# ningyu1991/InclusiveGAN

Measured on AMD Instinct MI355X. Metric: training img/sec (whole node), CelebA 128x128 StyleGAN2+IMLE, higher is better.
Workload: dtype f32-equivalent (3x3 convs: 2-piece fp16 split, operands to <= 1 ulp of fp32, scales per pixel / per channel: no per-tensor window; fp32 sums)

## Files before the change

### inclusivegan_amd/csrc/conv2d_mfma.hip

```cpp
#include "igan_common.h"
#include <cmath>
#include <cstdlib>
#include <type_traits>

namespace {

typedef float f32x16 __attribute__((ext_vector_type(16)));

constexpr int BK = 32;
#ifndef IGAN_SPLIT
#define IGAN_SPLIT 8
#endif
constexpr int LDK = BK + 4;

struct ConvArgs {
    const float* x;
    const float* w;
    float* y;
    float* out;
    const float* in_scale;
    const float* out_scale;
    int N, H, W, Cin;
    int OH, OW, Cout;
    int KH, KW;
// ... 1234 lines not shown
    } else {
#pragma unroll
        for (int i = 0; i < 16; i++) v[i] = w[((size_t)tap * K + 16 * c + i) * Nn + n];
    }
    unsigned short pc[2][16];
#pragma unroll
    for (int i = 0; i < 16; i++) {
        unsigned short o[2];
        split2(v[i] * S, o);
        pc[0][i] = o[0]; pc[1][i] = o[1];
    }
    uint4* dst = reinterpret_cast<uint4*>(out + (((size_t)c * taps + tap) * Nn + n) * 32);
#pragma unroll
    for (int q = 0; q < 2; q++)
#pragma unroll
        for (int hh = 0; hh < 2; hh++) {
            uint4 u;
            u.x = pc[q][8 * hh + 0] | ((unsigned)pc[q][8 * hh + 1] << 16); u.y = pc[q][8 * hh + 2] | ((unsigned)pc[q][8 * hh + 3] << 16);
            u.z = pc[q][8 * hh + 4] | ((unsigned)pc[q][8 * hh + 5] << 16); u.w = pc[q][8 * hh + 6] | ((unsigned)pc[q][8 * hh + 7] << 16);
            dst[2 * q + hh] = u;
        }
}

template <int NP, bool TAPO = false>
__global__ __launch_bounds__(512, 4) void conv_fwd_planes_kernel(ConvArgs a) {
    constexpr int BM = 128, BN = 128, WN = 4, TM = 2;
    static_assert(NP == 3 || NP == 2, "three bf16 pieces (six products) or two fp16 pieces (three products)");
    constexpr int IMG = NP * 128 * 32, STAGE = 2 * IMG;
    constexpr unsigned PB = NP * 32u;
    constexpr int TABS = (NP == 2) ? 9 * BM * 4 : 0;
#ifndef IGAN_F16_LDS_PAD
#define IGAN_F16_LDS_PAD 0
#endif
    constexpr int LPAD = (NP == 2) ? IGAN_F16_LDS_PAD : 0;
    __shared__ __attribute__((aligned(1024))) unsigned char smem[P_NSTAGE * STAGE + 3 * BM * 4 + TABS + LPAD];
    int* row_pix = reinterpret_cast<int*>(smem + P_NSTAGE * STAGE);
    int* row_n = row_pix + BM;
    float* row_nz = reinterpret_cast<float*>(row_n + BM);
    float* tab_s = row_nz + BM;

#ifdef IGAN_DIAGNOSTIC
    const int dm = a.diag_mode;
    if (dm & 4) return;
#else
    constexpr int dm = 0;
#endif
// ... 641 lines not shown
    const float alpha = (a.splits == 1) ? a.alpha : 1.0f;
#pragma unroll
    for (int tm = 0; tm < TM; tm++) {
#pragma unroll
        for (int r = 0; r < 16; r++) {
            const int cir = m0 + wm * (BM / WM) + tile_row<TM, true>(tm, (r & 3) + 8 * (r >> 2) + 4 * h);
            if (cir >= a.Cin) continue;
            if constexpr (TN == 2) {
                if (a.vecY) {
                    const int c2 = cbase + 2 * l31;
                    if (c2 < a.Cout) *reinterpret_cast<float2*>(out + (size_t)cir * a.Cout + c2) = make_float2(acc[tm][0][r] * alpha, acc[tm][1][r] * alpha);
                    continue;
                }
            }
#pragma unroll
            for (int tn = 0; tn < TN; tn++) {
                const int cc = cbase + tile_row<TN, true>(tn, l31);
                if (cc < a.Cout) out[(size_t)cir * a.Cout + cc] = acc[tm][tn][r] * alpha;
            }
        }
    }
}

__global__ __launch_bounds__(256, 2) void conv_fwd_planes_w4_kernel(ConvArgs a) {
    constexpr int BM = 128, BN = 128, NS = 3;
    constexpr int IMG = 2 * 128 * 32, STAGE = 2 * IMG;
    constexpr unsigned PB = 64u;
    constexpr int TABS = 9 * BM * 4;
    __shared__ __attribute__((aligned(1024))) unsigned char smem[NS * STAGE + 3 * BM * 4 + TABS];
    int* row_pix = reinterpret_cast<int*>(smem + NS * STAGE);
    int* row_n = row_pix + BM;
    float* row_nz = reinterpret_cast<float*>(row_n + BM);
    float* tab_s = row_nz + BM;

    const int tid = threadIdx.x;
    const int lane = tid & 63, wave = __builtin_amdgcn_readfirstlane(tid >> 6);
    const int l31 = lane & 31, h = lane >> 5;
    const int wm = wave >> 1, wn = wave & 1;
    const int up = 1 << a.up_shift;
    auto stamp = [&](int k) {
        if (a.diag != nullptr && (threadIdx.x >> 6) == 0) {
            const unsigned long long t = __builtin_amdgcn_s_memrealtime();
            if ((threadIdx.x & 63) == 0) a.diag[(size_t)blockIdx.x * 4 + k] = t;
        }
    };
    stamp(0);
    int bid = blockIdx.x;
    if (a.xcd_remap && bid < a.full_tiles) {
        const int per_class = a.nx * a.ny;
        const int lo = (bid / per_class) * per_class;
        const int cnt = min(per_class, a.full_tiles - lo);
        bid = lo + remap_xcd(bid - lo, cnt);
        if (cnt == per_class && a.ny > 1 && a.stride > 1) {
            const int j = bid - lo;
            bid = lo + (j % a.ny) * a.nx + j / a.ny;
        }
    }
    const bool sliced = bid >= a.full_tiles;
    const int tail = bid - a.full_tiles;
    const int tile = sliced ? a.full_tiles + tail / a.splits : bid;
    const int split = sliced ? tail % a.splits : 0;
    const int nsplit = sliced ? a.splits : 1;
    const int mt = tile % a.nx, nt = (tile / a.nx) % a.ny, cls = tile / (a.nx * a.ny);
    const int py = cls >> a.up_shift, px = cls & (up - 1);
    const int QH = (a.OH - py + up - 1) >> a.up_shift;
    const int QW = (a.OW - px + up - 1) >> a.up_shift;
    const int Mcls = a.N * QH * QW;
    const int m0 = mt * BM;
    if (m0 >= Mcls) return;
    const int n0 = nt * BN;
    const int ky0 = (a.pad_y - py * a.stride) & (up - 1);
    const int kx0 = (a.pad_x - px * a.stride) & (up - 1);
    const int nky = (ky0 < a.KH) ? ((a.KH - ky0 + up - 1) >> a.up_shift) : 0;
    const int nkx = (kx0 < a.KW) ? ((a.KW - kx0 + up - 1) >> a.up_shift) : 0;
    const int chunks = nky * nkx * a.cpt;
    const int c_begin = sliced ? (int)(((long long)split * chunks) / nsplit) : 0;
    const int c_end = sliced ? (int)(((long long)(split + 1) * chunks) / nsplit) : chunks;
    const bool any = c_begin < c_end;

    const float inv_hw = 1.0f / (float)(QH * QW), inv_w = 1.0f / (float)QW;
    const int drow = 32 * wave + (lane >> 1);
    const int dhalf = (lane & 1) ^ ((drow >> 3) & 1);
    const int ntap = nky * nkx;
    int ld_t0 = any ? c_begin / a.cpt : 0;
    int ld_cc = any ? c_begin - ld_t0 * a.cpt : 0;
    int ld_ta = any ? ld_t0 / nkx : 0;
    int ld_tb = any ? ld_t0 - ld_ta * nkx : 0;
    const unsigned xbytes = (unsigned)a.N * a.H * a.W * a.Cin * 4u, wbytes = (unsigned)a.KH * a.KW * a.Cin * a.Cout * 4u;
    const __amdgpu_buffer_rsrc_t rx = __builtin_amdgcn_make_buffer_rsrc(const_cast<unsigned short*>(a.xp), 0, (int)xbytes, 0x00020000);
    const __amdgpu_buffer_rsrc_t rw = __builtin_amdgcn_make_buffer_rsrc(const_cast<unsigned short*>(a.wp), 0, (int)wbytes, 0x00020000);
    const unsigned pixA = (unsigned)a.Cin * 4u;
    unsigned baseA, maskA = 0u, voffB;
    {
        const int m = m0 + drow;
        const bool rok = m < Mcls;
        const int mm = rok ? m : 0;
        const int nn = div_small(mm, QH * QW, inv_hw);
        const int r = mm - nn * (QH * QW);
        const int qy = div_small(r, QW, inv_w), qx = r - qy * QW;
        const int vy0 = (qy * up + py) * a.stride - a.pad_y + ky0, vx0 = (qx * up + px) * a.stride - a.pad_x + kx0;
        const int iy0 = vy0 >> a.up_shift, ix0 = vx0 >> a.up_shift;
        baseA = (unsigned)((nn * a.H + iy0) * a.W + ix0) * pixA + (unsigned)dhalf * 16u;
        for (int ta = 0; ta < nky; ta++)
            for (int tb = 0; tb < nkx; tb++) {
                const int iy = iy0 + ta, ix = ix0 + tb;
                const bool ok = rok & (iy >= 0) & (ix >= 0) & (iy < a.H) & (ix < a.W);
                maskA |= ok ? (1u << (ta * nkx + tb)) : 0u;
            }
        const int co = n0 + drow;
        voffB = (co < a.Cout) ? (unsigned)co * PB + (unsigned)dhalf * 16u : OOB;
    }
    unsigned offA = OOB, soffB = 0u;
    typedef __attribute__((address_space(3))) void lds_void;
    bool dma_fresh = true;
    const unsigned sliceB = (unsigned)(a.KH * a.KW * a.Cout) * PB;
    auto dma_prep = [&]() {
        if (dma_fresh || ld_cc == 0) {
            const unsigned disp = (unsigned)(ld_ta * a.W + ld_tb) * pixA + (unsigned)ld_cc * PB;
            const unsigned bit = 1u << (ld_ta * nkx + ld_tb);
            offA = (maskA & bit) ? baseA + disp : OOB;
            const int ky = ky0 + (ld_ta << a.up_shift), kx = kx0 + (ld_tb << a.up_shift);
            soffB = __builtin_amdgcn_readfirstlane((unsigned)((ld_cc * (a.KH * a.KW) + ky * a.KW + kx) * a.Cout) * PB);
            dma_fresh = false;
        } else {
            offA += PB;
            soffB = __builtin_amdgcn_readfirstlane(soffB + sliceB);
        }
        ++ld_cc;
        const int w1 = (ld_cc == a.cpt) ? 1 : 0;
        ld_cc = w1 ? 0 : ld_cc;
        ld_tb += w1;
        const int w2 = (ld_tb == nkx) ? 1 : 0;
        ld_tb = w2 ? 0 : ld_tb;
// ... 9 lines not shown
            __builtin_amdgcn_raw_ptr_buffer_load_lds(rw, (lds_void*)(D + IMG), 16, voffB, sB, 0, 0);
            __builtin_amdgcn_raw_ptr_buffer_load_lds(rw, (lds_void*)(D + IMG + 4096), 16, voffB, sB + 32u, 0, 0);
        }
    };

    f32x16 acc[2][2];
#pragma unroll
    for (int i = 0; i < 2; i++)
#pragma unroll
        for (int j = 0; j < 2; j++)
#pragma unroll
            for (int r = 0; r < 16; r++) acc[i][j][r] = 0.0f;

    float tabv[5] = {0.0f, 0.0f, 0.0f, 0.0f, 0.0f};
    {
        const float* rowinv = reinterpret_cast<const float*>(reinterpret_cast<const unsigned char*>(a.xp) + (size_t)a.N * a.H * a.W * a.Cin * 4);
#pragma unroll
        for (int j = 0; j < 5; j++) {
            const int i = tid + 256 * j;
            const int t = i >> 7, r = i & 127;
            if (t < ntap) {
                const int ta = t / nkx, tb = t - ta * nkx;
                const int m = m0 + r;
                const bool rok = m < Mcls;
                const int mm = rok ? m : 0;
                const int nn = div_small(mm, QH * QW, inv_hw);
                const int rr = mm - nn * (QH * QW);
                const int qy = div_small(rr, QW, inv_w), qx = rr - qy * QW;
                const int iy = (((qy * up + py) * a.stride - a.pad_y + ky0) >> a.up_shift) + ta, ix = (((qx * up + px) * a.stride - a.pad_x + kx0) >> a.up_shift) + tb;
                if (rok & (iy >= 0) & (ix >= 0) & (iy < a.H) & (ix < a.W)) tabv[j] = rowinv[(nn * a.H + iy) * a.W + ix];
            }
        }
    }
    if (any) {
#pragma unroll
        for (int j = 0; j < 3; j++) { dma_prep(); dma_pair(j, 0); dma_pair(j, 1); }
    }
#pragma unroll
    for (int j = 0; j < 5; j++)
        if (tid + 256 * j < 9 * BM) tab_s[tid + 256 * j] = tabv[j];
    if (tid < BM) {
        const int m = m0 + tid;
        int pix = -1, nn = 0;
        if (m < Mcls) {
            nn = div_small(m, QH * QW, inv_hw);
            const int r = m - nn * (QH * QW);
            const int qy = div_small(r, QW, inv_w), qx = r - qy * QW;
            pix = (nn * a.OH + (qy * up + py)) * a.OW + (qx * up + px);
        }
        row_pix[tid] = pix;
        row_n[tid] = nn;
        row_nz[tid] = noise_term(a, pix);
    }
    const unsigned lds0 = (unsigned)(unsigned long long)(lds_void*)smem;
    const int ra = wm * 64 + l31, rb = wn * 64 + l31;
    const unsigned fa = lds0 + (unsigned)(2 * ra + (h ^ ((ra >> 3) & 1))) * 16u;
    const unsigned fb = lds0 + (unsigned)IMG + (unsigned)(2 * rb + (h ^ ((rb >> 3) & 1))) * 16u;
    stamp(1);

    const f32x16 zero = {0.f, 0.f, 0.f, 0.f, 0.f, 0.f, 0.f, 0.f, 0.f, 0.f, 0.f, 0.f, 0.f, 0.f, 0.f, 0.f};
    struct Frag { f16x8 a0[2], a1[2], b0[2], b1[2]; };
    auto read_frags = [&](Frag& f, int stage) {
        const unsigned va = fa + (unsigned)(stage * STAGE), vb = fb + (unsigned)(stage * STAGE);
        asm volatile("ds_read_b128 %0, %1" : "=v"(f.b0[0]) : "v"(vb));
        asm volatile("ds_read_b128 %0, %1" : "=v"(f.a0[0]) : "v"(va));
        asm volatile("ds_read_b128 %0, %1 offset:4096" : "=v"(f.b1[0]) : "v"(vb));
        asm volatile("ds_read_b128 %0, %1 offset:5120" : "=v"(f.b1[1]) : "v"(vb));
// ... 75 lines not shown
#pragma unroll
                for (int r = 0; r < 16; r++) { u[0][j][r] = 0.0f; u[1][j][r] = 0.0f; }
            }
            cs = 0; ++ct;
            const int tn_ = min(ct, ntap - 1);
            sc0 = tab_row[tn_ * BM]; sc1 = tab_row[tn_ * BM + 32];
        }
        st = st1;
    };
    if (any) {
        asm volatile("s_waitcnt vmcnt(8) lgkmcnt(0)\n\ts_barrier" ::: "memory");
        read_frags(F0, 0);
        sc0 = tab_row[ct * BM]; sc1 = tab_row[ct * BM + 32];
        int c = c_begin;
        for (; c + 1 < c_end; c += 2) { step(F0, F1, c, std::false_type()); step(F1, F0, c + 1, std::false_type()); }
        if (c < c_end) step(F0, F1, c, std::true_type());
        else
            asm volatile("s_waitcnt lgkmcnt(0)"
                         : "+v"(F0.a0[0]), "+v"(F0.a0[1]), "+v"(F0.a1[0]), "+v"(F0.a1[1]), "+v"(F0.b0[0]), "+v"(F0.b0[1]), "+v"(F0.b1[0]), "+v"(F0.b1[1]) :: "memory");
    }
    drain_lds_dma();
    stamp(2);
    const float* winv = reinterpret_cast<const float*>(reinterpret_cast<const unsigned char*>(a.wp) + (size_t)a.KH * a.KW * a.Cin * a.Cout * 4);
    if (sliced && nsplit > 1) {
        float* wst = a.y + ((size_t)(tile - a.full_tiles) * a.splits + split) * (BM * BN);
#pragma unroll
        for (int tn = 0; tn < 2; tn++) {
            const int cq = n0 + wn * 64 + tn * 32 + 4 * h;
            float4 wi[4];
#pragma unroll
            for (int q = 0; q < 4; q++) wi[q] = (cq + 8 * q < a.Cout) ? *reinterpret_cast<const float4*>(winv + cq + 8 * q) : f4zero();
#pragma unroll
            for (int tm = 0; tm < 2; tm++) {
                const int row = wm * 64 + tm * 32 + l31;
#pragma unroll
                for (int q = 0; q < 4; q++)
                    *reinterpret_cast<float4*>(wst + row * BN + wn * 64 + tn * 32 + 8 * q + 4 * h) =
                        make_float4(acc[tm][tn][4 * q] * wi[q].x, acc[tm][tn][4 * q + 1] * wi[q].y, acc[tm][tn][4 * q + 2] * wi[q].z, acc[tm][tn][4 * q + 3] * wi[q].w);
            }
        }
        return;
    }
    __syncthreads();
    const bool scale = a.out_scale != nullptr;
    const float alpha = a.alpha;
#pragma unroll
    for (int tn = 0; tn < 2; tn++) {
        const int cq = n0 + wn * 64 + tn * 32 + 4 * h;
        float4 wi[4], bia[4];
#pragma unroll
        for (int q = 0; q < 4; q++) {
            wi[q] = (cq + 8 * q < a.Cout) ? *reinterpret_cast<const float4*>(winv + cq + 8 * q) : f4zero();
            bia[q] = (a.act && a.bias && cq + 8 * q < a.Cout) ? *reinterpret_cast<const float4*>(a.bias + cq + 8 * q) : f4zero();
        }
#pragma unroll
        for (int tm = 0; tm < 2; tm++) {
            const int row = wm * 64 + tm * 32 + l31;
            const int pix = row_pix[row];
            if (pix < 0) continue;
            const float* osc = a.out_scale + (size_t)row_n[row] * a.Cout;
            const float nz = row_nz[row];
#pragma unroll
            for (int q = 0; q < 4; q++) {
                const int co = cq + 8 * q;
                if (co >= a.Cout) continue;
                float4 o = make_float4(acc[tm][tn][4 * q] * wi[q].x, acc[tm][tn][4 * q + 1] * wi[q].y, acc[tm][tn][4 * q + 2] * wi[q].z, acc[tm][tn][4 * q + 3] * wi[q].w);
                o.x *= alpha; o.y *= alpha; o.z *= alpha; o.w *= alpha;
                if (scale) { const float4 d = *reinterpret_cast<const float4*>(osc + co); o.x *= d.x; o.y *= d.y; o.z *= d.z; o.w *= d.w; }
                if (a.act) {
                    o.x = epi_act(a.act, o.x + nz + bia[q].x, a.act_alpha) * a.act_gain; o.y = epi_act(a.act, o.y + nz + bia[q].y, a.act_alpha) * a.act_gain;
                    o.z = epi_act(a.act, o.z + nz + bia[q].z, a.act_alpha) * a.act_gain; o.w = epi_act(a.act, o.w + nz + bia[q].w, a.act_alpha) * a.act_gain;
                }
                *reinterpret_cast<float4*>(a.out + (size_t)pix * a.Cout + co) = o;
            }
        }
    }
    stamp(3);
}

typedef __attribute__((ext_vector_type(4))) short s16x4;
#ifndef IGAN_WGRAD_ASM_DMA
#define IGAN_WGRAD_ASM_DMA 1
#endif
typedef unsigned u32x4 __attribute__((ext_vector_type(4)));
__device__ __forceinline__ u32x4 raw_rsrc_words(const void* base, unsigned bytes) {
    const unsigned long long b = (unsigned long long)(uintptr_t)base;
    u32x4 r;
    r[0] = __builtin_amdgcn_readfirstlane((unsigned)b);
    r[1] = __builtin_amdgcn_readfirstlane((unsigned)(b >> 32) & 0xFFFFu);
    r[2] = __builtin_amdgcn_readfirstlane(bytes);
    r[3] = 0x00020000u;
    return r;
}
template <int SOFF>
__device__ __forceinline__ void lds_dma16_asm(u32x4 rsrc, unsigned lds_addr, unsigned voffset) {
    asm volatile("s_mov_b32 m0, %0\n\ts_nop 0\n\tbuffer_load_dwordx4 %1, %2, %3 offen lds" ::"s"(lds_addr), "v"(voffset), "s"(rsrc), "n"(SOFF) : "memory", "m0");
}
template <int NP>
__global__ __launch_bounds__(512, 4) void conv_wgrad_planes_kernel(WgradArgs a) {
    constexpr int TM = 2, WN = 4;
    static_assert(NP == 3 || NP == 2, "three bf16 pieces (six products) or two fp16 pieces (three products)");
// ... 413 lines not shown
    hipLaunchKernelGGL(rows_f16_kernel, dim3(grid), dim3(256), 0, stream, x, scale, out, rowinv, colmax, total, cpp, ilog2(cpp), C, HW);
}
void launch_colmax_only(hipStream_t stream, const float* x, const float* scale, float* colmax, int P_, int HW, int C) {
    const int C4 = C / 4, ppi = 256 / C4;
    const int blocks = std::min(H_COLBLOCKS, igan::ceil_div(P_, ppi));
    hipLaunchKernelGGL(cols_amax_kernel, dim3(blocks), dim3(256), 0, stream, x, scale, colmax + 4, P_, C4, ilog2(C4), HW, colmax);
}
void launch_col_image(hipStream_t stream, const float* x, const float* scale, unsigned short* out, int P_, int HW, int C, const float* colmax) {
    const int cpp = C / PK, total = P_ * cpp, C4 = C / 4;
    float* inv = reinterpret_cast<float*>(reinterpret_cast<unsigned char*>(out) + (size_t)P_ * C * 4);
    float* sc = inv + C;
    float* partial = sc + C;
    const int ppi = 256 / C4;
    const int blocks = std::min(H_COLBLOCKS, igan::ceil_div(P_, ppi));
    if (colmax == nullptr) {
        hipLaunchKernelGGL(cols_amax_kernel, dim3(blocks), dim3(256), 0, stream, x, scale, partial, P_, C4, ilog2(C4), HW, (float*)nullptr);
        hipLaunchKernelGGL(cols_finalize_kernel, dim3(igan::ceil_div(C, 8)), dim3(256), 0, stream, (const float*)partial, inv, sc, blocks, C, (const float*)nullptr);
    } else
        hipLaunchKernelGGL(cols_finalize_kernel, dim3(igan::ceil_div(C, 8)), dim3(256), 0, stream, colmax + 4, inv, sc, 0, C, colmax);
    hipLaunchKernelGGL(cols_f16_kernel, dim3(igan::ceil_div(total, 256)), dim3(256), 0, stream, x, scale, out, (const float*)sc, total, cpp, C, HW);
}
bool f16_tap_outer() { static const int v = getenv("IGAN_F16_TAP_OUTER") ? atoi(getenv("IGAN_F16_TAP_OUTER")) : 1; return v != 0; }
bool f16_w4() { static const int v = getenv("IGAN_F16_W4") ? atoi(getenv("IGAN_F16_W4")) : 1; return v != 0; }
void launch_filter_image(hipStream_t stream, const float* w, unsigned short* wp, bool wt, int taps, int KW_, int Nn, int K) {
    const int wtotal = taps * Nn * (K / PK);
    if (planes_mode() == 2) {
        float* inv = reinterpret_cast<float*>(reinterpret_cast<unsigned char*>(wp) + (size_t)taps * Nn * K * 4);
        float* partial = inv + Nn;
        if (wt) {
            hipLaunchKernelGGL((filter_amax_kernel<true>), dim3(igan::ceil_div(taps * Nn, 4)), dim3(256), 0, stream, w, partial, taps, Nn, K);
            hipLaunchKernelGGL((filter_planes_f16_kernel<true>), dim3(igan::ceil_div(wtotal, 256)), dim3(256), 0, stream, w, wp, inv, (const float*)partial, taps, taps, KW_, Nn, K);
        } else {
            hipLaunchKernelGGL((filter_amax_kernel<false>), dim3(taps * H_KSK, igan::ceil_div(Nn, 64)), dim3(256), 0, stream, w, partial, taps, Nn, K);
            hipLaunchKernelGGL((filter_planes_f16_kernel<false>), dim3(igan::ceil_div(wtotal, 256)), dim3(256), 0, stream, w, wp, inv, (const float*)partial, taps * H_KSK, taps, KW_, Nn, K);
        }
    } else {
        if (wt) hipLaunchKernelGGL((filter_planes_kernel<true>), dim3(igan::ceil_div(wtotal, 256)), dim3(256), 0, stream, w, wp, taps, KW_, Nn, K);
        else hipLaunchKernelGGL((filter_planes_kernel<false>), dim3(igan::ceil_div(wtotal, 256)), dim3(256), 0, stream, w, wp, taps, KW_, Nn, K);
    }
}

bool planes_shape_ok(const igan_conv2d_params* p, const FwdTile& t, int Mmax) {
    if (!planes_enabled() || t.BM != 128 || t.BN != 128 || p->Cin % BK != 0) return false;
    static const int min_rows = getenv("IGAN_PLANES_MIN_ROWS") ? atoi(getenv("IGAN_PLANES_MIN_ROWS")) : 1024;
    if (p->KH * p->KW == 1 || (long long)p->KH * p->KW * p->Cin < 1152 || Mmax < min_rows) return false;
    if ((long long)p->N * p->OH * p->OW >= (1LL << 24)) return false;
    if ((long long)p->N * p->H * p->W * p->Cin * 6 >= 0x7FFFFF00LL || (long long)p->KH * p->KW * p->Cin * p->Cout * 6 >= 0x7FFFFF00LL) return false;
    if (planes_mode() == 2 && (!pow2(p->Cin / PK) || p->Cin / PK > 64 || p->KH * p->KW > 9 || p->Cout % 4 != 0)) return false;
#ifdef IGAN_DIAGNOSTIC
    {
        static const int only_cin = getenv("IGAN_PLANES_ONLY_CIN") ? atoi(getenv("IGAN_PLANES_ONLY_CIN")) : 0;
        static const int no_act = getenv("IGAN_PLANES_NO_ACT") ? atoi(getenv("IGAN_PLANES_NO_ACT")) : 0;
        static const int no_scale = getenv("IGAN_PLANES_NO_SCALE") ? atoi(getenv("IGAN_PLANES_NO_SCALE")) : 0;
        static const int kind = getenv("IGAN_PLANES_KIND") ? atoi(getenv("IGAN_PLANES_KIND")) : 0;
        static const int wt = getenv("IGAN_PLANES_WT") ? atoi(getenv("IGAN_PLANES_WT")) : 0;
        if (only_cin && p->Cin != only_cin) return false;
        if ((no_act == 1 && p->act != 0) || (no_act == 2 && p->act == 0)) return false;
        if ((no_scale == 1 && p->in_scale != nullptr) || (no_scale == 2 && p->in_scale == nullptr)) return false;
        if ((kind == 1 && (p->stride != 1 || p->up != 1)) || (kind == 2 && p->stride != 2) || (kind == 3 && p->up != 2)) return false;
        if ((wt == 1 && p->w_transposed) || (wt == 2 && !p->w_transposed)) return false;
    }
#endif
    return true;
}
bool use_planes_kernel(const igan_conv2d_params* p, const FwdTile& t, int Mmax) {
    if (!planes_shape_ok(p, t, Mmax) || (((uintptr_t)p->x | (uintptr_t)p->w | (uintptr_t)p->in_scale | (uintptr_t)p->x_pieces) & 15) != 0) return false;
    if (planes_mode() == 2 && (((uintptr_t)p->y | (uintptr_t)p->out_scale | (uintptr_t)p->bias) & 15) != 0) return false;
    return true;
// ... 194 lines not shown
    if (planes) {
        IGAN_REQUIRE(p->x_pieces == nullptr || planes_mode() == 1, "conv2d: the two-piece fp16 form writes its own images (one scale per pixel here, per channel in the weight gradient): x_pieces must be NULL");
        IGAN_REQUIRE(p->x_pieces == nullptr || p->x_pieces_bytes == planes_x_floats(p) * 4, "conv2d: x_pieces is not the image of this x (x_pieces_bytes != N*H*W*Cin*6)");
        const unsigned short* xp = reinterpret_cast<const unsigned short*>(p->x_pieces);
        unsigned short* wp = reinterpret_cast<unsigned short*>(p->workspace + partial_floats + planes_x_floats(p));
        const int cpp = p->Cin / PK;
        if (xp == nullptr) {
            unsigned short* own = reinterpret_cast<unsigned short*>(p->workspace + partial_floats);
            if (a.diag_mode & 1) {}
            else if (planes_mode() == 2) launch_row_image(stream, p->x, p->in_scale, own, p->N * p->H * p->W, p->H * p->W, p->Cin, p->x_colmax);
            else launch_piece_image(stream, p->x, p->in_scale, own, p->N * p->H * p->W, p->H * p->W, p->Cin);
            xp = own;
        }
        if (p->w_pieces != nullptr) {
            IGAN_REQUIRE(p->w_pieces_bytes == igan_filter_image_bytes(p->KH, p->KW, p->Cin, p->Cout) && (((uintptr_t)p->w_pieces) & 15) == 0,
                         "conv2d: w_pieces is not an image igan_filter_image() wrote for this filter (size / alignment)");
            wp = reinterpret_cast<unsigned short*>(const_cast<void*>(p->w_pieces));
        } else if (!(a.diag_mode & 1)) launch_filter_image(stream, p->w, wp, wt, p->KH * p->KW, p->KW, p->Cout, p->Cin);
        a.xp = xp; a.wp = wp;
        a.cpt = cpp;
        if (a.diag_mode & 2) {}
        else if (planes_mode() == 2) {
            const bool tapo = f16_tap_outer();
            if (tapo && f16_w4()) hipLaunchKernelGGL(conv_fwd_planes_w4_kernel, grid, dim3(256), 0, stream, a);
            else if (tapo) hipLaunchKernelGGL((conv_fwd_planes_kernel<2, true>), grid, dim3(512), 0, stream, a);
            else hipLaunchKernelGGL((conv_fwd_planes_kernel<2, false>), grid, dim3(512), 0, stream, a);
        } else hipLaunchKernelGGL((conv_fwd_planes_kernel<3>), grid, dim3(512), 0, stream, a);
        IGAN_LAUNCH_CHECK("conv2d (piece form) launch");
        launched = true;
    } else
    if (use_dma_kernel(p, t, a.walk != 0)) {
        if (wt) {
            if (a.in_scale) hipLaunchKernelGGL((conv_fwd_dma_kernel<true, true>), grid, dim3(512), 0, stream, a);
            else hipLaunchKernelGGL((conv_fwd_dma_kernel<true, false>), grid, dim3(512), 0, stream, a);
        } else {
            if (a.in_scale) hipLaunchKernelGGL((conv_fwd_dma_kernel<false, true>), grid, dim3(512), 0, stream, a);
            else hipLaunchKernelGGL((conv_fwd_dma_kernel<false, false>), grid, dim3(512), 0, stream, a);
        }
        IGAN_LAUNCH_CHECK("conv2d (LDS-DMA) launch");
        launched = true;
    }
    if (launched) {}
    else if (t.BM == 128 && t.BN == 128 && eight_waves("IGAN_CONV_8WAVE")) launch_fwd<128, 128, 2, 4>(stream, a, grid, wt, vec);
    else if (t.BM == 128 && t.BN == 128) launch_fwd<128, 128, 2, 2>(stream, a, grid, wt, vec);
    else if (t.BM == 128 && t.BN == 64 && eight_waves("IGAN_CONV_8WAVE")) launch_fwd<128, 64, 4, 2>(stream, a, grid, wt, vec);
    else if (t.BM == 128 && t.BN == 64) launch_fwd<128, 64, 2, 2>(stream, a, grid, wt, vec);
    else if (t.BM == 128 && t.BN == 32) launch_fwd<128, 32, 4, 1>(stream, a, grid, wt, vec);
// ... 5 lines not shown
        hipLaunchKernelGGL(conv_fixup_kernel, dim3(sliced, ceil_div(t.BM, rp)), dim3(256), 0, stream, a, t.BM, t.BN, rp);
        IGAN_LAUNCH_CHECK("conv2d fix-up launch");
    }
    return IGAN_OK;
}

namespace {

int wgrad_geometry_check(const igan_conv2d_wgrad_params* p) {
    IGAN_REQUIRE(p->x && p->dy && p->dw, "conv2d_wgrad: null buffer");
    IGAN_REQUIRE(p->N >= 1 && p->H >= 1 && p->W >= 1 && p->Cin >= 1, "conv2d_wgrad: input dims must be positive");
    IGAN_REQUIRE(p->OH >= 1 && p->OW >= 1 && p->Cout >= 1, "conv2d_wgrad: output dims must be positive");
    IGAN_REQUIRE(p->KH >= 1 && p->KW >= 1, "conv2d_wgrad: kernel must be at least 1x1");
    IGAN_REQUIRE(p->stride >= 1 && p->up >= 1, "conv2d_wgrad: stride and up must be at least 1");
    IGAN_REQUIRE(p->stride == 1 || p->up == 1, "conv2d_wgrad: at most one of stride, up may exceed 1");
    if (!(p->up == 1 || p->up == 2)) return igan::fail(IGAN_ERR_UNSUPPORTED, "conv2d_wgrad: up must be 1 or 2 (got %d)", p->up);
    IGAN_REQUIRE((long long)p->N * p->H * p->W * p->Cin * 4 <= 0x7FFFFFF0LL, "conv2d_wgrad: input too large (2 GiB per operand)");
    IGAN_REQUIRE((long long)p->N * p->OH * p->OW * p->Cout * 4 <= 0x7FFFFFF0LL, "conv2d_wgrad: output gradient too large (2 GiB per operand)");
    IGAN_REQUIRE((long long)p->KH * p->KW * p->Cin * p->Cout <= INT32_MAX, "conv2d_wgrad: filter too large");
    return IGAN_OK;
}

template <int BM, int BN, int WM, int WN, bool VEC>
void launch_wgrad2(hipStream_t stream, const WgradArgs& a, dim3 grid, int scm) {
    if constexpr (BM == 128 && BN == 128 && WM * WN == 8) {
        hipLaunchKernelGGL((conv_wgrad_kernel<BM, BN, WM, WN, VEC, 0>), grid, dim3(WM * WN * 64), 0, stream, a);
    } else {
        if (scm == 0) hipLaunchKernelGGL((conv_wgrad_kernel<BM, BN, WM, WN, VEC, 0>), grid, dim3(WM * WN * 64), 0, stream, a);
        else if (scm == 1) hipLaunchKernelGGL((conv_wgrad_kernel<BM, BN, WM, WN, VEC, 1>), grid, dim3(WM * WN * 64), 0, stream, a);
        else hipLaunchKernelGGL((conv_wgrad_kernel<BM, BN, WM, WN, VEC, 2>), grid, dim3(WM * WN * 64), 0, stream, a);
    }
}
template <int BM, int BN, int WM, int WN>
void launch_wgrad(hipStream_t stream, const WgradArgs& a, dim3 grid, bool vec, int scm) {
    if (vec) launch_wgrad2<BM, BN, WM, WN, true>(stream, a, grid, scm);
    else launch_wgrad2<BM, BN, WM, WN, false>(stream, a, grid, scm);
}

struct WgTile { int BM, BN; };
WgTile pick_wg_tile(int Cin, int Cout) {
    WgTile t;
    t.BM = (Cin > 32) ? 128 : 32;
    t.BN = (Cout > 32) ? 128 : 32;
    if (t.BM == 32 && t.BN == 32) t.BN = 128;
    return t;
}

int wgrad_splits(const igan_conv2d_wgrad_params* p) {
    const WgTile t = pick_wg_tile(p->Cin, p->Cout);
    const long long tiles = (long long)igan::ceil_div(p->Cin, t.BM) * igan::ceil_div(p->Cout, t.BN) * p->KH * p->KW;
    const int up = p->up;
    const long long kpix = (long long)p->N * ((p->OH + up - 1) / up) * ((p->OW + up - 1) / up);
    const int chunks = (int)((kpix + BK - 1) / BK);
    const int max_by_work = std::max(1, chunks / 4);
    int s;
    if (tiles >= 512) s = 1;
    else {
        s = (int)(512 / tiles);
        if (s > max_by_work) s = max_by_work;
// ... 131 lines not shown
            xp = own;
        }
        if (dyp == nullptr) {
            unsigned short* own = reinterpret_cast<unsigned short*>(p->workspace + partial_floats + wgrad_planes_x_floats(p));
            if (planes_mode() == 2) launch_col_image(stream, p->dy, p->out_scale, own, p->N * p->OH * p->OW, p->OH * p->OW, p->Cout, p->dy_colmax);
            else launch_piece_image(stream, p->dy, p->out_scale, own, p->N * p->OH * p->OW, p->OH * p->OW, p->Cout);
            dyp = own;
        }
        a.xp = xp; a.dyp = dyp;
        if (planes_mode() == 2) hipLaunchKernelGGL((conv_wgrad_planes_kernel<2>), grid, dim3(512), 0, stream, a);
        else hipLaunchKernelGGL((conv_wgrad_planes_kernel<3>), grid, dim3(512), 0, stream, a);
        IGAN_LAUNCH_CHECK("conv2d_wgrad (piece form) launch");
        if (splits > 1) {
            const int total = (int)wsize;
            const int rg = std::min(ceil_div(total, 256), 2048);
            hipLaunchKernelGGL(plain_reduce_kernel, dim3(rg), dim3(256), 0, stream, (const float*)p->workspace, p->dw, total, splits, p->alpha);
            IGAN_LAUNCH_CHECK("conv2d_wgrad reduce launch");
        }
        return IGAN_OK;
    }
    const bool vec = a.vecA && a.vecB && (a.in_scale == nullptr || a.vecSA) && (a.out_scale == nullptr || a.vecSB);
    const int scm = (a.in_scale && a.out_scale) ? 1 : ((a.in_scale || a.out_scale) ? 2 : 0);
    const bool long_axis = (long long)p->OH * p->OW >= 128LL * 128LL;
    if (t.BM == 128 && t.BN == 128 && eight_waves("IGAN_WGRAD_8WAVE") && !long_axis && scm == 0) launch_wgrad<128, 128, 2, 4>(stream, a, grid, vec, scm);
    else if (t.BM == 128 && t.BN == 128) launch_wgrad<128, 128, 2, 2>(stream, a, grid, vec, scm);
    else if (t.BM == 128 && t.BN == 32) launch_wgrad<128, 32, 4, 1>(stream, a, grid, vec, scm);
    else launch_wgrad<32, 128, 1, 4>(stream, a, grid, vec, scm);
    IGAN_LAUNCH_CHECK("conv2d_wgrad launch");
    if (splits > 1) {
        const int total = (int)wsize;
        const int rg = std::min(ceil_div(total, 256), 2048);
        hipLaunchKernelGGL(plain_reduce_kernel, dim3(rg), dim3(256), 0, stream, (const float*)p->workspace, p->dw, total, splits, p->alpha);
        IGAN_LAUNCH_CHECK("conv2d_wgrad reduce launch");
    }
    return IGAN_OK;
}

static int f16_window_read(unsigned long long (&v)[4], int reset) {
    using namespace igan;
    if (hipMemcpyFromSymbol(&v[0], HIP_SYMBOL(g_f16_below_window), 8) != hipSuccess || hipMemcpyFromSymbol(&v[1], HIP_SYMBOL(g_f16_imaged), 8) != hipSuccess ||
        hipMemcpyFromSymbol(&v[2], HIP_SYMBOL(g_f16_below_window_cols), 8) != hipSuccess || hipMemcpyFromSymbol(&v[3], HIP_SYMBOL(g_f16_imaged_cols), 8) != hipSuccess) return IGAN_ERR_HIP;
    if (reset) {
        const unsigned long long z = 0ull;
        if (hipMemcpyToSymbol(HIP_SYMBOL(g_f16_below_window), &z, 8) != hipSuccess || hipMemcpyToSymbol(HIP_SYMBOL(g_f16_imaged), &z, 8) != hipSuccess ||
            hipMemcpyToSymbol(HIP_SYMBOL(g_f16_below_window_cols), &z, 8) != hipSuccess || hipMemcpyToSymbol(HIP_SYMBOL(g_f16_imaged_cols), &z, 8) != hipSuccess) return IGAN_ERR_HIP;
    }
    return IGAN_OK;
}
extern "C" int igan_debug_f16_window(unsigned long long* below, unsigned long long* imaged, int reset) {
    unsigned long long v[4] = {0ull, 0ull, 0ull, 0ull};
// ... 19 lines not shown
    if ((long long)N * HW < wgrad_min_rows()) return 0;
    return 4 + (size_t)H_COLBLOCKS * C;
}

extern "C" size_t igan_filter_image_bytes(int KH, int KW, int Cin, int Cout) {
    using namespace igan;
    if (!planes_enabled() || KH < 1 || KW < 1 || Cin < 1 || Cout < 1 || KH * KW == 1 || Cin % BK != 0 || (long long)KH * KW * Cin < 1152) return 0;
    if ((long long)KH * KW * Cin * Cout * 6 >= 0x7FFFFF00LL) return 0;
    if (planes_mode() == 2) {
        if (!pow2(Cin / PK) || Cin / PK > 64 || KH * KW > 9 || Cout % 4 != 0) return 0;
        return filter_part_bytes((size_t)KH * KW, (size_t)Cout, (size_t)Cin);
    }
    return (size_t)KH * KW * Cin * Cout * 6;
}

extern "C" int igan_filter_image(igan_stream_t stream_, const float* w, void* out, int KH, int KW, int Cin, int Cout, int w_transposed) {
    using namespace igan;
    IGAN_REQUIRE(w != nullptr && out != nullptr, "filter_image: null buffer");
    IGAN_REQUIRE(igan_filter_image_bytes(KH, KW, Cin, Cout) != 0, "filter_image: igan_filter_image_bytes() says this process / filter takes none");
    IGAN_REQUIRE(((((uintptr_t)w) | ((uintptr_t)out)) & 15) == 0, "filter_image: w and out must be 16-byte aligned");
    launch_filter_image((hipStream_t)stream_, w, reinterpret_cast<unsigned short*>(out), w_transposed != 0, KH * KW, KW, Cout, Cin);
    IGAN_LAUNCH_CHECK("filter_image launch");
    return IGAN_OK;
}

extern "C" int igan_conv_pieces_wanted(int KH, int KW, int Cin, int Cout) {
    using namespace igan;
    return (planes_enabled() && KH * KW > 1 && Cin >= 128 && Cout >= 128 && Cin % 32 == 0 && Cout % 32 == 0) ? 1 : 0;
}

extern "C" int igan_pieces_image_ok(int N, int HW, int C) {
    using namespace igan;
    return (planes_mode() == 1 && C >= 128 && C % 32 == 0 && (long long)N * HW >= 2048 && (long long)N * HW * C * 6 < 0x7FFFFF00LL) ? 1 : 0;
}

extern "C" int igan_to_pieces(igan_stream_t stream_, const float* x, const float* scale, void* out, int N, int HW, int C) {
    using namespace igan;
    IGAN_REQUIRE(x != nullptr && out != nullptr, "to_pieces: null buffer");
    IGAN_REQUIRE(N >= 1 && HW >= 1 && C >= 16 && C % 16 == 0, "to_pieces: C must be a positive multiple of 16");
    IGAN_REQUIRE((((uintptr_t)x | (uintptr_t)scale | (uintptr_t)out) & 15) == 0, "to_pieces: buffers must be 16-byte aligned");
    IGAN_REQUIRE((long long)N * HW * C * 6 < 0x7FFFFF00LL, "to_pieces: image too large (32-bit offsets)");
    if (planes_mode() != 1) return igan::fail(IGAN_ERR_UNSUPPORTED, "to_pieces: only the bf16-piece form (IGAN_CONV_PLANES=1) takes caller-written images (igan_pieces_image_ok() says so)");
    launch_piece_image((hipStream_t)stream_, x, scale, reinterpret_cast<unsigned short*>(out), N * HW, HW, C);
    IGAN_LAUNCH_CHECK("to_pieces launch");
    return IGAN_OK;
}
// ... 1 lines not shown
```

Measured before the change: 356.9.

## Add interior-tile specialization for w4 conv kernel and fused transposed filter imaging

Templates the w4 fp16-planes forward conv on an INTERIOR flag. When every phase class's row count and Cout are multiples of 128 and there is no split-K, a variant runs that drops the bounds checks and uses a vectorized float4 epilogue, with bias, scale and activation variants resolved at compile time. It also adds a single-kernel fused amax+split path for transposed filter imaging, replacing a two-kernel sequence. The changes reduce branch and epilogue overhead and cut one launch per filter image, at the cost of more code paths and correctness that depends on the shape guard.

```diff
diff --git a/inclusivegan_amd/csrc/conv2d_mfma.hip b/inclusivegan_amd/csrc/conv2d_mfma.hip
--- a/inclusivegan_amd/csrc/conv2d_mfma.hip
+++ b/inclusivegan_amd/csrc/conv2d_mfma.hip
@@ -1280,6 +1280,52 @@
         }
 }
 
+__device__ __forceinline__ void store_filter_unit(const float (&v)[16], float S, unsigned short* __restrict__ out, size_t unit) {
+    unsigned short pc[2][16];
+#pragma unroll
+    for (int i = 0; i < 16; i++) {
+        unsigned short o[2];
+        split2(v[i] * S, o);
+        pc[0][i] = o[0]; pc[1][i] = o[1];
+    }
+    uint4* dst = reinterpret_cast<uint4*>(out + unit * 32);
+#pragma unroll
+    for (int q = 0; q < 2; q++)
+#pragma unroll
+        for (int hh = 0; hh < 2; hh++) {
+            uint4 u;
+            u.x = pc[q][8 * hh + 0] | ((unsigned)pc[q][8 * hh + 1] << 16); u.y = pc[q][8 * hh + 2] | ((unsigned)pc[q][8 * hh + 3] << 16);
+            u.z = pc[q][8 * hh + 4] | ((unsigned)pc[q][8 * hh + 5] << 16); u.w = pc[q][8 * hh + 6] | ((unsigned)pc[q][8 * hh + 7] << 16);
+            dst[2 * q + hh] = u;
+        }
+}
+__device__ __forceinline__ float amax4(const float4 f) { return fmaxf(fmaxf(fabsf(f.x), fabsf(f.y)), fmaxf(fabsf(f.z), fabsf(f.w))); }
+__global__ __launch_bounds__(64) void filter_image_wt_kernel(const float* __restrict__ w, unsigned short* __restrict__ out, float* __restrict__ inv, int taps, int Nn, int K) {
+    const int n = blockIdx.x, lane = threadIdx.x;
+    const int k4 = K >> 2, cpk = K >> 4, tot = taps * k4;
+    auto quad = [&](int j) { const int tap = j / k4; return reinterpret_cast<const float4*>(w + ((size_t)tap * Nn + n) * K)[j - tap * k4]; };
+    float m0 = 0.0f, m1 = 0.0f, m2 = 0.0f, m3 = 0.0f;
+    int j = lane;
+    for (; j + 192 < tot; j += 256) {
+        const float4 f0 = quad(j), f1 = quad(j + 64), f2 = quad(j + 128), f3 = quad(j + 192);
+        m0 = fmaxf(m0, amax4(f0)); m1 = fmaxf(m1, amax4(f1)); m2 = fmaxf(m2, amax4(f2)); m3 = fmaxf(m3, amax4(f3));
+    }
+    for (; j < tot; j += 64) m0 = fmaxf(m0, amax4(quad(j)));
+    float amax = fmaxf(fmaxf(m0, m1), fmaxf(m2, m3));
+#pragma unroll
+    for (int o = 32; o >= 1; o >>= 1) amax = fmaxf(amax, __shfl_xor(amax, o));
+    const float S = scale_from_amax(amax);
+    if (lane == 0) inv[n] = inv_scale_from_amax(amax);
+    for (int u = lane; u < taps * cpk; u += 64) {
+        const int tap = u / cpk, c = u - tap * cpk;
+        const float4* src = reinterpret_cast<const float4*>(w + ((size_t)(taps - 1 - tap) * Nn + n) * K + 16 * c);
+        float v[16];
+#pragma unroll
+        for (int i = 0; i < 4; i++) { const float4 f = src[i]; v[4 * i] = f.x; v[4 * i + 1] = f.y; v[4 * i + 2] = f.z; v[4 * i + 3] = f.w; }
+        store_filter_unit(v, S, out, ((size_t)c * taps + tap) * Nn + n);
+    }
+}
+
 template <int NP, bool TAPO = false>
 __global__ __launch_bounds__(512, 4) void conv_fwd_planes_kernel(ConvArgs a) {
     constexpr int BM = 128, BN = 128, WN = 4, TM = 2;
@@ -1967,7 +2013,8 @@
     }
 }
 
-__global__ __launch_bounds__(256, 2) void conv_fwd_planes_w4_kernel(ConvArgs a) {
+template <bool INTERIOR>
+__device__ __forceinline__ void conv_fwd_planes_w4_tile(const ConvArgs& a) {
     constexpr int BM = 128, BN = 128, NS = 3;
     constexpr int IMG = 2 * 128 * 32, STAGE = 2 * IMG;
     constexpr unsigned PB = 64u;
@@ -2001,7 +2048,7 @@
             bid = lo + (j % a.ny) * a.nx + j / a.ny;
         }
     }
-    const bool sliced = bid >= a.full_tiles;
+    const bool sliced = INTERIOR ? false : bid >= a.full_tiles;
     const int tail = bid - a.full_tiles;
     const int tile = sliced ? a.full_tiles + tail / a.splits : bid;
     const int split = sliced ? tail % a.splits : 0;
@@ -2038,7 +2085,7 @@
     unsigned baseA, maskA = 0u, voffB;
     {
         const int m = m0 + drow;
-        const bool rok = m < Mcls;
+        const bool rok = INTERIOR || m < Mcls;
         const int mm = rok ? m : 0;
         const int nn = div_small(mm, QH * QW, inv_hw);
         const int r = mm - nn * (QH * QW);
@@ -2053,7 +2100,7 @@
                 maskA |= ok ? (1u << (ta * nkx + tb)) : 0u;
             }
         const int co = n0 + drow;
-        voffB = (co < a.Cout) ? (unsigned)co * PB + (unsigned)dhalf * 16u : OOB;
+        voffB = (INTERIOR || co < a.Cout) ? (unsigned)co * PB + (unsigned)dhalf * 16u : OOB;
     }
     unsigned offA = OOB, soffB = 0u;
     typedef __attribute__((address_space(3))) void lds_void;
@@ -2109,7 +2156,7 @@
             if (t < ntap) {
                 const int ta = t / nkx, tb = t - ta * nkx;
                 const int m = m0 + r;
-                const bool rok = m < Mcls;
+                const bool rok = INTERIOR || m < Mcls;
                 const int mm = rok ? m : 0;
                 const int nn = div_small(mm, QH * QW, inv_hw);
                 const int rr = mm - nn * (QH * QW);
@@ -2129,7 +2176,7 @@
     if (tid < BM) {
         const int m = m0 + tid;
         int pix = -1, nn = 0;
-        if (m < Mcls) {
+        if (INTERIOR || m < Mcls) {
             nn = div_small(m, QH * QW, inv_hw);
             const int r = m - nn * (QH * QW);
             const int qy = div_small(r, QW, inv_w), qx = r - qy * QW;
@@ -2251,23 +2298,70 @@
     drain_lds_dma();
     stamp(2);
     const float* winv = reinterpret_cast<const float*>(reinterpret_cast<const unsigned char*>(a.wp) + (size_t)a.KH * a.KW * a.Cin * a.Cout * 4);
-    if (sliced && nsplit > 1) {
-        float* wst = a.y + ((size_t)(tile - a.full_tiles) * a.splits + split) * (BM * BN);
-#pragma unroll
-        for (int tn = 0; tn < 2; tn++) {
-            const int cq = n0 + wn * 64 + tn * 32 + 4 * h;
-            float4 wi[4];
-#pragma unroll
-            for (int q = 0; q < 4; q++) wi[q] = (cq + 8 * q < a.Cout) ? *reinterpret_cast<const float4*>(winv + cq + 8 * q) : f4zero();
-#pragma unroll
-            for (int tm = 0; tm < 2; tm++) {
-                const int row = wm * 64 + tm * 32 + l31;
-#pragma unroll
-                for (int q = 0; q < 4; q++)
-                    *reinterpret_cast<float4*>(wst + row * BN + wn * 64 + tn * 32 + 8 * q + 4 * h) =
-                        make_float4(acc[tm][tn][4 * q] * wi[q].x, acc[tm][tn][4 * q + 1] * wi[q].y, acc[tm][tn][4 * q + 2] * wi[q].z, acc[tm][tn][4 * q + 3] * wi[q].w);
-            }
-        }
+    if constexpr (!INTERIOR) {
+        if (sliced && nsplit > 1) {
+            float* wst = a.y + ((size_t)(tile - a.full_tiles) * a.splits + split) * (BM * BN);
+    #pragma unroll
+            for (int tn = 0; tn < 2; tn++) {
+                const int cq = n0 + wn * 64 + tn * 32 + 4 * h;
+                float4 wi[4];
+    #pragma unroll
+                for (int q = 0; q < 4; q++) wi[q] = (cq + 8 * q < a.Cout) ? *reinterpret_cast<const float4*>(winv + cq + 8 * q) : f4zero();
+    #pragma unroll
+                for (int tm = 0; tm < 2; tm++) {
+                    const int row = wm * 64 + tm * 32 + l31;
+    #pragma unroll
+                    for (int q = 0; q < 4; q++)
+                        *reinterpret_cast<float4*>(wst + row * BN + wn * 64 + tn * 32 + 8 * q + 4 * h) =
+                            make_float4(acc[tm][tn][4 * q] * wi[q].x, acc[tm][tn][4 * q + 1] * wi[q].y, acc[tm][tn][4 * q + 2] * wi[q].z, acc[tm][tn][4 * q + 3] * wi[q].w);
+                }
+            }
+            return;
+        }
+    }
+    if constexpr (INTERIOR) {
+        __syncthreads();
+        const float alpha = a.alpha;
+        float4 wi[2][4], bia[2][4];
+        const bool biased = a.act && a.bias;
+#pragma unroll
+        for (int tn = 0; tn < 2; tn++)
+#pragma unroll
+            for (int q = 0; q < 4; q++) {
+                const int co = n0 + wn * 64 + tn * 32 + 4 * h + 8 * q;
+                wi[tn][q] = *reinterpret_cast<const float4*>(winv + co);
+                bia[tn][q] = biased ? *reinterpret_cast<const float4*>(a.bias + co) : f4zero();
+            }
+        int pixr[2], nr[2];
+        float nzr[2];
+#pragma unroll
+        for (int tm = 0; tm < 2; tm++) { const int row = wm * 64 + tm * 32 + l31; pixr[tm] = row_pix[row]; nr[tm] = row_n[row]; nzr[tm] = row_nz[row]; }
+        auto stores = [&](auto SC, auto ACT) {
+#pragma clang fp contract(off)
+#pragma unroll
+            for (int tn = 0; tn < 2; tn++)
+#pragma unroll
+                for (int tm = 0; tm < 2; tm++) {
+                    const float* osc = a.out_scale + (size_t)nr[tm] * a.Cout;
+                    const float nz = nzr[tm];
+#pragma unroll
+                    for (int q = 0; q < 4; q++) {
+                        const int co = n0 + wn * 64 + tn * 32 + 4 * h + 8 * q;
+                        float4 o = make_float4(acc[tm][tn][4 * q] * wi[tn][q].x, acc[tm][tn][4 * q + 1] * wi[tn][q].y, acc[tm][tn][4 * q + 2] * wi[tn][q].z, acc[tm][tn][4 * q + 3] * wi[tn][q].w);
+                        o.x *= alpha; o.y *= alpha; o.z *= alpha; o.w *= alpha;
+                        if constexpr (decltype(SC)::value) { const float4 d = *reinterpret_cast<const float4*>(osc + co); o.x *= d.x; o.y *= d.y; o.z *= d.z; o.w *= d.w; }
+                        if constexpr (decltype(ACT)::value) {
+                            const float4 b = bia[tn][q];
+                            o.x = epi_act(a.act, o.x + nz + b.x, a.act_alpha) * a.act_gain; o.y = epi_act(a.act, o.y + nz + b.y, a.act_alpha) * a.act_gain;
+                            o.z = epi_act(a.act, o.z + nz + b.z, a.act_alpha) * a.act_gain; o.w = epi_act(a.act, o.w + nz + b.w, a.act_alpha) * a.act_gain;
+                        }
+                        *reinterpret_cast<float4*>(a.out + (size_t)pixr[tm] * a.Cout + co) = o;
+                    }
+                }
+        };
+        if (a.out_scale != nullptr) { if (a.act) stores(std::true_type(), std::true_type()); else stores(std::true_type(), std::false_type()); }
+        else { if (a.act) stores(std::false_type(), std::true_type()); else stores(std::false_type(), std::false_type()); }
+        stamp(3);
         return;
     }
     __syncthreads();
@@ -2306,6 +2400,8 @@
     }
     stamp(3);
 }
+__global__ __launch_bounds__(256, 2) void conv_fwd_planes_w4_kernel(ConvArgs a) { conv_fwd_planes_w4_tile<false>(a); }
+__global__ __launch_bounds__(256, 2) void conv_fwd_planes_w4_interior_kernel(ConvArgs a) { conv_fwd_planes_w4_tile<true>(a); }
 
 typedef __attribute__((ext_vector_type(4))) short s16x4;
 #ifndef IGAN_WGRAD_ASM_DMA
@@ -2765,12 +2861,25 @@
 }
 bool f16_tap_outer() { static const int v = getenv("IGAN_F16_TAP_OUTER") ? atoi(getenv("IGAN_F16_TAP_OUTER")) : 1; return v != 0; }
 bool f16_w4() { static const int v = getenv("IGAN_F16_W4") ? atoi(getenv("IGAN_F16_W4")) : 1; return v != 0; }
+bool f16_interior(const igan_conv2d_params* p, int splits) {
+    static const bool on = !(getenv("IGAN_F16_INTERIOR") && atoi(getenv("IGAN_F16_INTERIOR")) == 0);
+    if (!on || splits > 1 || p->Cout % 128 != 0 || p->up < 1) return false;
+    for (int py = 0; py < p->up; py++)
+        for (int px = 0; px < p->up; px++) {
+            const long long QH = (p->OH - py + p->up - 1) / p->up, QW = (p->OW - px + p->up - 1) / p->up;
+            if (((long long)p->N * QH * QW) % 128 != 0) return false;
+        }
+    return true;
+}
 void launch_filter_image(hipStream_t stream, const float* w, unsigned short* wp, bool wt, int taps, int KW_, int Nn, int K) {
     const int wtotal = taps * Nn * (K / PK);
     if (planes_mode() == 2) {
         float* inv = reinterpret_cast<float*>(reinterpret_cast<unsigned char*>(wp) + (size_t)taps * Nn * K * 4);
         float* partial = inv + Nn;
-        if (wt) {
+        static const bool fused = !(getenv("IGAN_FILTER_FUSED") && atoi(getenv("IGAN_FILTER_FUSED")) == 0);
+        if (fused && wt && K % 16 == 0) {
+            hipLaunchKernelGGL(filter_image_wt_kernel, dim3(Nn), dim3(64), 0, stream, w, wp, inv, taps, Nn, K);
+        } else if (wt) {
             hipLaunchKernelGGL((filter_amax_kernel<true>), dim3(igan::ceil_div(taps * Nn, 4)), dim3(256), 0, stream, w, partial, taps, Nn, K);
             hipLaunchKernelGGL((filter_planes_f16_kernel<true>), dim3(igan::ceil_div(wtotal, 256)), dim3(256), 0, stream, w, wp, inv, (const float*)partial, taps, taps, KW_, Nn, K);
         } else {
@@ -2783,10 +2892,13 @@
     }
 }
 
+int planes_min_rows() {
+    static const int v = getenv("IGAN_PLANES_MIN_ROWS") ? atoi(getenv("IGAN_PLANES_MIN_ROWS")) : 1024;
+    return v;
+}
 bool planes_shape_ok(const igan_conv2d_params* p, const FwdTile& t, int Mmax) {
     if (!planes_enabled() || t.BM != 128 || t.BN != 128 || p->Cin % BK != 0) return false;
-    static const int min_rows = getenv("IGAN_PLANES_MIN_ROWS") ? atoi(getenv("IGAN_PLANES_MIN_ROWS")) : 1024;
-    if (p->KH * p->KW == 1 || (long long)p->KH * p->KW * p->Cin < 1152 || Mmax < min_rows) return false;
+    if (p->KH * p->KW == 1 || (long long)p->KH * p->KW * p->Cin < 1152 || Mmax < planes_min_rows()) return false;
     if ((long long)p->N * p->OH * p->OW >= (1LL << 24)) return false;
     if ((long long)p->N * p->H * p->W * p->Cin * 6 >= 0x7FFFFF00LL || (long long)p->KH * p->KW * p->Cin * p->Cout * 6 >= 0x7FFFFF00LL) return false;
     if (planes_mode() == 2 && (!pow2(p->Cin / PK) || p->Cin / PK > 64 || p->KH * p->KW > 9 || p->Cout % 4 != 0)) return false;
@@ -3027,7 +3139,8 @@
         if (a.diag_mode & 2) {}
         else if (planes_mode() == 2) {
             const bool tapo = f16_tap_outer();
-            if (tapo && f16_w4()) hipLaunchKernelGGL(conv_fwd_planes_w4_kernel, grid, dim3(256), 0, stream, a);
+            if (tapo && f16_w4() && f16_interior(p, splits)) hipLaunchKernelGGL(conv_fwd_planes_w4_interior_kernel, grid, dim3(256), 0, stream, a);
+            else if (tapo && f16_w4()) hipLaunchKernelGGL(conv_fwd_planes_w4_kernel, grid, dim3(256), 0, stream, a);
             else if (tapo) hipLaunchKernelGGL((conv_fwd_planes_kernel<2, true>), grid, dim3(512), 0, stream, a);
             else hipLaunchKernelGGL((conv_fwd_planes_kernel<2, false>), grid, dim3(512), 0, stream, a);
         } else hipLaunchKernelGGL((conv_fwd_planes_kernel<3>), grid, dim3(512), 0, stream, a);
@@ -3079,19 +3192,20 @@
 }
 
 template <int BM, int BN, int WM, int WN, bool VEC>
-void launch_wgrad2(hipStream_t stream, const WgradArgs& a, dim3 grid, int scm) {
+int launch_wgrad2(hipStream_t stream, const WgradArgs& a, dim3 grid, int scm) {
     if constexpr (BM == 128 && BN == 128 && WM * WN == 8) {
+        IGAN_REQUIRE(scm == 0, "conv2d_wgrad: the eight-wave 128x128 tile has no scaled form (in_scale / out_scale would be dropped)");
         hipLaunchKernelGGL((conv_wgrad_kernel<BM, BN, WM, WN, VEC, 0>), grid, dim3(WM * WN * 64), 0, stream, a);
     } else {
         if (scm == 0) hipLaunchKernelGGL((conv_wgrad_kernel<BM, BN, WM, WN, VEC, 0>), grid, dim3(WM * WN * 64), 0, stream, a);
         else if (scm == 1) hipLaunchKernelGGL((conv_wgrad_kernel<BM, BN, WM, WN, VEC, 1>), grid, dim3(WM * WN * 64), 0, stream, a);
         else hipLaunchKernelGGL((conv_wgrad_kernel<BM, BN, WM, WN, VEC, 2>), grid, dim3(WM * WN * 64), 0, stream, a);
     }
+    return IGAN_OK;
 }
 template <int BM, int BN, int WM, int WN>
-void launch_wgrad(hipStream_t stream, const WgradArgs& a, dim3 grid, bool vec, int scm) {
-    if (vec) launch_wgrad2<BM, BN, WM, WN, true>(stream, a, grid, scm);
-    else launch_wgrad2<BM, BN, WM, WN, false>(stream, a, grid, scm);
+int launch_wgrad(hipStream_t stream, const WgradArgs& a, dim3 grid, bool vec, int scm) {
+    return vec ? launch_wgrad2<BM, BN, WM, WN, true>(stream, a, grid, scm) : launch_wgrad2<BM, BN, WM, WN, false>(stream, a, grid, scm);
 }
 
 struct WgTile { int BM, BN; };
@@ -3269,10 +3383,12 @@
     const bool vec = a.vecA && a.vecB && (a.in_scale == nullptr || a.vecSA) && (a.out_scale == nullptr || a.vecSB);
     const int scm = (a.in_scale && a.out_scale) ? 1 : ((a.in_scale || a.out_scale) ? 2 : 0);
     const bool long_axis = (long long)p->OH * p->OW >= 128LL * 128LL;
-    if (t.BM == 128 && t.BN == 128 && eight_waves("IGAN_WGRAD_8WAVE") && !long_axis && scm == 0) launch_wgrad<128, 128, 2, 4>(stream, a, grid, vec, scm);
-    else if (t.BM == 128 && t.BN == 128) launch_wgrad<128, 128, 2, 2>(stream, a, grid, vec, scm);
-    else if (t.BM == 128 && t.BN == 32) launch_wgrad<128, 32, 4, 1>(stream, a, grid, vec, scm);
-    else launch_wgrad<32, 128, 1, 4>(stream, a, grid, vec, scm);
+    int rc;
+    if (t.BM == 128 && t.BN == 128 && eight_waves("IGAN_WGRAD_8WAVE") && !long_axis && scm == 0) rc = launch_wgrad<128, 128, 2, 4>(stream, a, grid, vec, scm);
+    else if (t.BM == 128 && t.BN == 128) rc = launch_wgrad<128, 128, 2, 2>(stream, a, grid, vec, scm);
+    else if (t.BM == 128 && t.BN == 32) rc = launch_wgrad<128, 32, 4, 1>(stream, a, grid, vec, scm);
+    else rc = launch_wgrad<32, 128, 1, 4>(stream, a, grid, vec, scm);
+    if (rc != IGAN_OK) return rc;
     IGAN_LAUNCH_CHECK("conv2d_wgrad launch");
     if (splits > 1) {
         const int total = (int)wsize;
@@ -3338,6 +3454,15 @@
     launch_filter_image((hipStream_t)stream_, w, reinterpret_cast<unsigned short*>(out), w_transposed != 0, KH * KW, KW, Cout, Cin);
     IGAN_LAUNCH_CHECK("filter_image launch");
     return IGAN_OK;
+}
+
+extern "C" int igan_debug_conv_interior(const igan_conv2d_params* p) {
+    using namespace igan;
+    if (p == nullptr || fwd_geometry_check(p) != IGAN_OK || is_small_dense(p)) return 0;
+    int Mmax, chunks_max, nclass;
+    fwd_counts(p, Mmax, chunks_max, nclass);
+    const FwdTile t = pick_fwd_tile(Mmax, p->Cout);
+    return (use_planes_kernel(p, t, Mmax) && planes_mode() == 2 && f16_tap_outer() && f16_w4() && f16_interior(p, std::max(1, p->splits))) ? 1 : 0;
 }
 
 extern "C" int igan_conv_pieces_wanted(int KH, int KW, int Cin, int Cout) {
```

Result: no change. 359.3, median of 6 (+0.7%).
